# kshedden/muscato

Hardware: AMD Instinct MI355X
Metric: reads/sec (100 bp, multi-map) at 1/2/4/8 MI355X; confirm-kernel HBM GB/s vs peak (higher is better)
Workload: dtype u32

## Files before the change

muscato_amd/build.py:

```python
from __future__ import annotations

import os
import shutil
import subprocess
from concurrent.futures import ThreadPoolExecutor

HERE = os.path.dirname(os.path.abspath(__file__))
CSRC = os.path.join(HERE, "csrc")
LIB = os.path.join(HERE, "libmuscato_hip.so")
OBJ = os.path.join(HERE, "build")
SOURCES = [os.path.join(CSRC, f) for f in ("muscato_hip.hip", "match_lane_rw4.hip", "match_lane_rw8.hip", "match_lane_rw12.hip",
                                           "match_lane_rw8w.hip", "match_lane_rw12w.hip", "match_lane_rw16w.hip", "match_lane_rw8s.hip", "match_dma_rw8.hip")]
HEADERS = [os.path.join(os.path.dirname(HERE), "include", "muscato_hip.h")] + \
    [os.path.join(CSRC, f) for f in sorted(os.listdir(CSRC)) if f.endswith(".hpp")]
LANE_ONLY = os.path.join(CSRC, "kernels_match_lane.hpp")
DMA_ONLY = os.path.join(CSRC, "kernels_match_dma.hpp")
FLAGS = ["--offload-arch=gfx950", "-O3", "-std=c++17", "-fPIC", "-Wall", "-Wno-unused-function"]


def hipcc() -> str:
    for cand in (shutil.which("hipcc"), "/opt/rocm/bin/hipcc"):
        if cand and os.path.exists(cand):
            return cand
    raise RuntimeError("hipcc not found: libmuscato_hip.so cannot be built")


def needs_build() -> bool:
    if not os.path.exists(LIB):
        return True
    t = os.path.getmtime(LIB)
    return any(os.path.getmtime(p) > t for p in SOURCES + HEADERS)


HOST = os.path.join(CSRC, "host")
BIN = os.path.join(HERE, "bin")
HOST_HEADERS = [os.path.join(HOST, f) for f in sorted(os.listdir(HOST)) if f.endswith(".hpp")]
TOOLS = {"muscato": "muscato_cli.cpp", "muscato_prep_targets": "muscato_prep_targets.cpp",
         "muscato_screen": "muscato_screen.cpp", "muscato_confirm": "muscato_confirm.cpp"}
GPU_TOOLS = ("muscato", "muscato_prep_targets", "muscato_screen", "muscato_confirm")


def build_tools(force: bool = False, verbose: bool = False) -> None:
    os.makedirs(BIN, exist_ok=True)
    for name, src in TOOLS.items():
        out = os.path.join(BIN, name)
        srcp = os.path.join(HOST, src)
        deps = [srcp] + HOST_HEADERS + HEADERS
        if not force and os.path.exists(out) and all(os.path.getmtime(d) <= os.path.getmtime(out) for d in deps):
            continue
        cmd = ["g++", "-O2", "-std=c++17", "-Wall", "-pthread", "-o", out, srcp, "-lz"]
        if name in GPU_TOOLS:
            cmd += ["-L" + HERE, "-lmuscato_hip", "-Wl,-rpath,$ORIGIN/.."]
        if verbose:
            print(" ".join(cmd))
        subprocess.check_call(cmd)


_API = "../../include/muscato_hip.h"
_HOST_CHAIN = ("host/muscato_host.hpp", "host/cli_config.hpp", "host/cli_maxmatches_host.hpp", "host/cli_names.hpp", "host/cli_plan.hpp",
               "host/cli_text.hpp", "host/sz.hpp", _API)
CHECKS = {
    "cli_plan_check": ("cli_plan_check.cpp", ("host/check.hpp", "host/cli_names.hpp", "host/cli_plan.hpp"), 83_615_609, ()),
    "ctx_state_check": ("ctx_state_check.cpp", ("host/check.hpp", "ctx_state.hpp", _API), 58_376_821, ()),
    "dev_mem_check": ("dev_mem_check.cpp", ("host/check.hpp", "dev_mem.hpp"), 492, ()),
    "index_plan_check": ("index_plan_check.cpp", ("host/check.hpp", "index_plan.hpp"), 567_030, ()),
    "load_plan_check": ("load_plan_check.cpp", ("host/check.hpp", "load_plan.hpp"), 35_240_767, ()),
    "maxmatches_plan_check": ("maxmatches_plan_check.cpp", ("host/check.hpp", "maxmatches_plan.hpp"), 548_365, ()),
    "read_names_plan_check": ("read_names_plan_check.cpp", ("host/check.hpp", "read_names_plan.hpp"), 21_577_989, ()),
    "side_names_check": ("side_names_check.cpp", ("host/check.hpp", "side_names.hpp"), 100_517, ()),
    "sz_plan_check": ("sz_plan_check.cpp", ("host/check.hpp", "sz_plan.hpp", "host/sz.hpp"), 3_599_466, ("-lz",)),
    "targets_prep_plan_check": ("targets_prep_plan_check.cpp", ("host/check.hpp", "sz_plan.hpp", "targets_prep_plan.hpp") + _HOST_CHAIN, 12_757_977, ("-lz",)),
    "text_stage_check": ("text_stage_check.cpp", ("host/check.hpp", "text_stage.hpp"), 1_711_086, ()),
}
SANITIZE = ["-O1", "-g", "-fsanitize=address,undefined", "-fno-sanitize-recover=all", "-static-libasan", "-static-libubsan"]


def check_headers(name: str) -> list:
    return [os.path.normpath(os.path.join(CSRC, h)) for h in CHECKS[name][1]]


def build_checks(force: bool = False, verbose: bool = False, sanitize: bool = False, out_dir: str = BIN) -> dict:
    os.makedirs(out_dir, exist_ok=True)

    def one(name: str) -> str:
        src, _, _, libs = CHECKS[name]
        out = os.path.join(out_dir, name + ("_san" if sanitize else ""))
        srcp = os.path.join(HOST, src)
        deps = [srcp] + check_headers(name)
        if force or not os.path.exists(out) or any(os.path.getmtime(d) > os.path.getmtime(out) for d in deps):
            cmd = ["g++", "-std=c++17", "-Wall"] + (SANITIZE if sanitize else ["-O2"]) + ["-o", out, srcp] + list(libs)
            if verbose:
                print(" ".join(cmd))
            subprocess.check_call(cmd)
        return out

    with ThreadPoolExecutor(max_workers=len(CHECKS)) as ex:
        return dict(zip(CHECKS, ex.map(one, CHECKS)))


def _compile(src: str, force: bool, verbose: bool, defines=(), tag: str = "") -> str:
    obj = os.path.join(OBJ, os.path.basename(src) + tag + ".o")
    base = os.path.basename(src)
    deps = [src] + [h for h in HEADERS if (h != LANE_ONLY or "match_lane" in base or "match_dma" in base) and (h != DMA_ONLY or "match_dma" in base)]
    if not force and os.path.exists(obj) and all(os.path.getmtime(d) <= os.path.getmtime(obj) for d in deps):
        return obj
    cmd = [hipcc()] + FLAGS + list(defines) + ["-c", "-o", obj, src]
    if verbose:
        print(" ".join(cmd))
    subprocess.check_call(cmd)
    return obj


def build(force: bool = False, verbose: bool = False) -> str:
    if force or needs_build():
        os.makedirs(OBJ, exist_ok=True)
        with ThreadPoolExecutor(max_workers=len(SOURCES)) as ex:
            objs = list(ex.map(lambda s: _compile(s, force, verbose), SOURCES))
        cmd = [hipcc(), "--offload-arch=gfx950", "-shared", "-fPIC", "-o", LIB] + objs + ["-ldl"]
        if verbose:
            print(" ".join(cmd))
        subprocess.check_call(cmd)
    build_tools(force=force, verbose=verbose)
    build_checks(force=force, verbose=verbose)
    return LIB


def variant(name: str, defines) -> str:
    os.makedirs(OBJ, exist_ok=True)
    out_dir = os.path.join(os.path.dirname(HERE), "build_variants")
    os.makedirs(out_dir, exist_ok=True)
    with ThreadPoolExecutor(max_workers=len(SOURCES)) as ex:
        main_defs = ["-D" + d[len("-DMAIN_"):] for d in defines if d.startswith("-DMAIN_")]
        lane_defs = [d for d in defines if not d.startswith("-DMAIN_")]
        objs = list(ex.map(lambda s: _compile(s, False, False, lane_defs if ("match_lane" in s or "match_dma" in s) else main_defs,
                                              "." + name if (("match_lane" in s or "match_dma" in s) and lane_defs) or ("match_lane" not in s and "match_dma" not in s and main_defs) else ""), SOURCES))
    out = os.path.join(out_dir, name + ".so")
    subprocess.check_call([hipcc(), "--offload-arch=gfx950", "-shared", "-fPIC", "-o", out] + objs + ["-ldl"])
    return out


if __name__ == "__main__":
    import sys
    if len(sys.argv) > 2 and sys.argv[1] == "variant":
        print(variant(sys.argv[2], sys.argv[3:]))
    else:
        print(build(force="--force" in sys.argv, verbose=True))
```

muscato_amd/csrc/muscato_hip.hip:

```cpp

#include <hip/hip_runtime.h>
#include <rccl/rccl.h>
#include <dlfcn.h>

#include <algorithm>
#include <cstdarg>
#include <cstdio>
#include <cstdlib>
#include <cstring>
#include <map>
#include <mutex>
#include <string>
#include <type_traits>
#include <vector>

#include "../../include/muscato_hip.h"

#include "ctx_state.hpp"
#include "dev_mem.hpp"
#include "index_plan.hpp"
#include "load_plan.hpp"

#include "kernels_common.hpp"
#include "kernels_index.hpp"
#include "kernels_screen.hpp"
#include "kernels_confirm.hpp"
#include "kernels_match.hpp"
#include "kernels_match_lane_inst.hpp"
#include "kernels_screen_lane.hpp"
#include "kernels_partition.hpp"
#include "kernels_results.hpp"
#include "side_names.hpp"
#include "kernels_side.hpp"
#include "kernels_maxmatches.hpp"
#include "kernels_fastq.hpp"
MUSC_LANE_INSTANCES_4(extern)
MUSC_LANE_INSTANCES_8(extern)
MUSC_LANE_INSTANCES_12(extern)
MUSC_LANE_INSTANCES_8W(extern)
MUSC_LANE_INSTANCES_12W(extern)
MUSC_LANE_INSTANCES_16W(extern)
MUSC_LANE_INSTANCES_SPEC(extern)
MUSC_DMA_INSTANCES(extern)


namespace {

thread_local std::string g_init_error;

struct Roctx {
  int (*push)(const char*) = nullptr;
  int (*pop)() = nullptr;
  Roctx() {
    for (const char* name : {"librocprofiler-sdk-roctx.so.1", "librocprofiler-sdk-roctx.so", "libroctx64.so.4", "libroctx64.so"}) {
      if (void* h = dlopen(name, RTLD_NOW | RTLD_LOCAL)) {
        push = reinterpret_cast<int (*)(const char*)>(dlsym(h, "roctxRangePushA"));
        pop = reinterpret_cast<int (*)()>(dlsym(h, "roctxRangePop"));
        if (push && pop) return;
        push = nullptr;
        pop = nullptr;
      }
    }
  }
};
const Roctx& roctx() {
  static const Roctx r;
  return r;
}
struct Range {
  bool on;
  explicit Range(const char* name) : on(roctx().push != nullptr) {
    if (on) (void)roctx().push(name);
  }
  ~Range() {
    if (on) (void)roctx().pop();
  }
};

struct CaptureGuard {
  hipStream_t st = nullptr;
  bool active = false;
  hipError_t begin(hipStream_t s) {
    const hipError_t e = hipStreamBeginCapture(s, hipStreamCaptureModeThreadLocal);
    if (e == hipSuccess) {
      st = s;
      active = true;
    }
    return e;
  }
  hipError_t end(hipGraph_t* g) {
    active = false;
    return hipStreamEndCapture(st, g);
  }
  ~CaptureGuard() {
    if (!active) return;
    hipGraph_t g = nullptr;
    (void)hipStreamEndCapture(st, &g);
    if (g) (void)hipGraphDestroy(g);
    (void)hipGetLastError();
  }
};

}

using musc_load::RecShape;
using musc_load::StreamPlan;
using musc_load::stream_plan;
using musc_load::stream_plan_batch;

struct EnvKnobs : musc_index::Knobs {
  bool match_dma = false;
  bool screen_wg = false;
  int context = 0;
  bool no_x_context = false;
  bool force_wide = false;
  int debug_grid = 0;
  bool debug_sync = false;
  int graph = -1;
  bool pipeline = false;
  bool no_spec = false;
  long batch_reads = 0;
  uint64_t stage_bytes = 64ull << 20;
  uint64_t stage_lines = 1ull << 20;
  long mm_heap_lds = 0;
  void read() {
    *this = EnvKnobs();
    auto is = [](const char* v, const char* w) { return v && !strcmp(v, w); };
    const char* e = getenv("MUSC_INDEX");
    index = is(e, "classic") ? musc_index::IDX_CLASSIC : is(e, "lines") ? musc_index::IDX_LINES : is(e, "classic64") ? musc_index::IDX_CLASSIC64 : musc_index::IDX_AUTO;
    e = getenv("MUSC_MATCH");
    match_dma = is(e, "dma");
    screen_wg = is(getenv("MUSC_SCREEN"), "wg");
    e = getenv("MUSC_CONTEXT");
    context = is(e, "narrow") ? 1 : is(e, "wide") ? 2 : 0;
    no_x_context = getenv("MUSC_NO_X_CONTEXT") != nullptr;
    force_wide = getenv("MUSC_DEBUG_FORCE_WIDE") != nullptr;
    if ((e = getenv("MUSC_DEBUG_INDEX_BITS"))) index_bits = atoi(e);
    ctx_direct = (e = getenv("MUSC_DEBUG_CTX_DIRECT")) && atoi(e) > 0;
    if ((e = getenv("MUSC_DEBUG_GRID"))) debug_grid = atoi(e);
    debug_sync = getenv("MUSC_DEBUG_SYNC") != nullptr;
    if ((e = getenv("MUSC_GRAPH"))) graph = atoi(e);
    if ((e = getenv("MUSC_PIPELINE"))) pipeline = atoi(e) > 0;
    no_spec = getenv("MUSC_NO_SPEC") != nullptr;
    if ((e = getenv("MUSC_BATCH_READS"))) batch_reads = atol(e);
    if ((e = getenv("MUSC_DEBUG_INDEX_BUDGET_MB"))) index_budget_mb = atol(e);
    if ((e = getenv("MUSC_DEBUG_STAGE_BYTES")) && atoll(e) > 0) stage_bytes = (uint64_t)atoll(e);
    if ((e = getenv("MUSC_DEBUG_STAGE_LINES")) && atoll(e) > 0) stage_lines = (uint64_t)atoll(e);
    if ((e = getenv("MUSC_DEBUG_MM_HEAP_LDS"))) mm_heap_lds = atol(e);
  }
};

struct musc_ctx {
  int device = 0;
  hipStream_t stream = nullptr;
  std::string err;
  EnvKnobs env;
  musc_state::State st;

  DevPtr<uint32_t> db2;
  DevPtr<uint32_t> dbm2;
  bool db_has_x = false;
  bool reads_have_x = false;
  DevBuf<uint32_t> rdx;
  struct { uint64_t gen = 0; int wide = -1; } rdx_of;
  struct { uint64_t gen = 0; double pmatch = -1.0; int32_t mmp1 = -1; bool ok = false; } xok;
  DevPtr<uint32_t> dbx;
  uint64_t max_tlen = 0;
  struct { uint64_t gen = 0; int32_t key[CTX_MAX_W + 3] = {0}; bool ok = false; } xokdb;
  DevPtr<uint64_t> seq_off;
  uint32_t nseq = 0;
  uint64_t nbases = 0;
  uint64_t db_words = 0;
  std::vector<uint64_t> h_seq_off;

  uint64_t part_bases = 0;
  std::vector<uint32_t> part_first;
  musc_index::Kind part_kind = musc_index::K_CLASSIC64;
  uint64_t part_size = 0;
  uint32_t cur_part = 0;
  DevBuf<musc_hit> pacc;
  DevBuf<uint32_t> pbest;
  DevBuf<uint64_t> pcnt, padj;
  DevBuf<uint32_t> pflags, pflags_tmp;
  DevBuf<uint32_t> block_acc;

  musc_index::Resident idx;
  int wide = 0;
  DevMem idx_T, idx_E, ctx_T, ctx_E;
  unsigned scrt_resident = 0;
  int scrt_rw = 0;
  uint64_t idx_novf = 0;
  DevPtr<PathParams> d_pp;
  PathParams h_pp;
  bool h_pp_valid = false;
  DevPtr<MatchParams> d_mp;
  MatchParams h_mp;
  bool h_mp_valid = false;
  int spec_geom = 0;
  DevBuf<uint4> spill;

  DevPtr<uint32_t> rd;
  uint64_t rd_cap = 0;
  DevPtr<uint32_t> rdm;
  uint64_t nreads = 0;
  int rw = 0;
  uint32_t max_len = 0;
  bool reads_failed = false;

  struct Upload {
    DevPtr<uint32_t> stage;
    hipStream_t s_up = nullptr;
    std::vector<hipEvent_t> ev;
    StreamPlan plan;
    uint64_t next_piece = 0;
    uint64_t packed_upto = 0;
    uint32_t L = 0;
    bool active = false;
  } up;

  struct BatchSet {
    DevBuf<uint32_t> wb, rvalid, tbase, tcount;
    DevBuf<uint4> cdesc;
  } bs[2];
  int cur = 0;
  hipStream_t stream2 = nullptr;
  hipStream_t s_confirm = nullptr;
  hipEvent_t ev_ready[2] = {nullptr, nullptr}, ev_free[2] = {nullptr, nullptr}, ev_join = nullptr;
  DevBuf<uint32_t> scan_tmp, tcount2, tpre;
  DevBuf<uint4> stage;
  DevBuf<uint32_t> p_nx;
  DevBuf<uint16_t> nmiss_tab;
// ... 1004 lines not shown
```

muscato_amd/csrc/muscato_prep.hpp:

```cpp

#include <rocprim/device/device_radix_sort.hpp>

#define PREP_BASES_PER_WORD 21

DEV uint32_t prep_code(unsigned char ch) {
  switch (ch) {
    case 'A': return 1u;
    case 'C': return 2u;
    case 'G': return 3u;
    case 'T': return 4u;
    default: return 5u;
  }
}

MUSC_KERNEL __launch_bounds__(256) void k_prep_keys(const unsigned char* __restrict__ s,
                                                   const uint64_t* __restrict__ off,
                                                   const uint32_t* __restrict__ perm, uint64_t n, uint32_t w,
                                                   uint64_t* __restrict__ keys) {
  for (uint64_t i = (uint64_t)blockIdx.x * blockDim.x + threadIdx.x; i < n; i += (uint64_t)gridDim.x * blockDim.x) {
    const uint32_t r = perm[i];
    const uint64_t o = off[r];
    const uint64_t len = off[r + 1] - o;
    const uint64_t first = (uint64_t)w * PREP_BASES_PER_WORD;
    uint64_t key = 0;
    for (uint32_t j = 0; j < PREP_BASES_PER_WORD; j++) {
      const uint64_t q = first + j;
      if (q >= len) break;
      key |= (uint64_t)prep_code(s[o + q]) << (60 - 3 * j);
    }
    keys[i] = key;
  }
}

MUSC_KERNEL void k_prep_iota(uint32_t* __restrict__ p, uint64_t n) {
  for (uint64_t i = (uint64_t)blockIdx.x * blockDim.x + threadIdx.x; i < n; i += (uint64_t)gridDim.x * blockDim.x)
    p[i] = (uint32_t)i;
}

MUSC_KERNEL __launch_bounds__(256) void k_prep_heads(const unsigned char* __restrict__ s,
                                                    const uint64_t* __restrict__ off,
                                                    const uint32_t* __restrict__ perm, uint64_t n,
                                                    uint32_t* __restrict__ head) {
  for (uint64_t i = (uint64_t)blockIdx.x * blockDim.x + threadIdx.x; i < n; i += (uint64_t)gridDim.x * blockDim.x) {
    uint32_t h = 1;
    if (i > 0) {
      const uint32_t a = perm[i], b = perm[i - 1];
      const uint64_t oa = off[a], ob = off[b];
      const uint64_t la = off[a + 1] - oa, lb = off[b + 1] - ob;
      if (la == lb) {
        h = 0;
        for (uint64_t q = 0; q < la; q++)
          if (s[oa + q] != s[ob + q]) {
            h = 1;
            break;
          }
      }
    }
    head[i] = h;
  }
}

MUSC_KERNEL void k_prep_starts(const uint32_t* __restrict__ head, const uint32_t* __restrict__ incl, uint64_t n,
                              uint32_t* __restrict__ ustart, uint32_t* __restrict__ uhead,
                              const uint32_t* __restrict__ perm) {
  for (uint64_t i = (uint64_t)blockIdx.x * blockDim.x + threadIdx.x; i < n; i += (uint64_t)gridDim.x * blockDim.x) {
    if (head[i]) {
      ustart[incl[i] - 1] = (uint32_t)i;
      uhead[incl[i] - 1] = perm[i];
    }
    if (i == n - 1) ustart[incl[i]] = (uint32_t)n;
  }
}

MUSC_KERNEL void k_prep_pack(const unsigned char* __restrict__ s, const uint64_t* __restrict__ off,
                            const uint32_t* __restrict__ uhead, uint64_t nunique, int rw,
                            uint32_t* __restrict__ rd, uint32_t* __restrict__ rdm, uint32_t* __restrict__ has_x) {
  const uint64_t t = (uint64_t)blockIdx.x * blockDim.x + threadIdx.x;
  const uint64_t g = t / rw;
  const int j = (int)(t % rw);
  if (g >= nunique) return;
  const uint32_t r = uhead[g];
  const uint64_t o = off[r];
  const uint32_t len = (uint32_t)(off[r + 1] - o);
  if (j == rw - 1) {
    uint32_t anyx = 0;
    for (uint32_t q = 0; q < len; q++) {
      uint32_t isx;
      (void)ascii_code(s[o + q], &isx);
      anyx |= isx;
    }
    rd[t] = (len & 0xFFFFu) | (anyx ? READ_HAS_X : 0u);
    rdm[t] = 0;
    return;
  }
  uint32_t v = 0, mv = 0;
  for (int b = 0; b < 16; b++) {
    const uint32_t q = (uint32_t)j * 16 + b;
    if (q < len) {
      uint32_t isx;
      const uint32_t c = ascii_code(s[o + q], &isx);
      v |= c << (2 * b);
      mv |= isx << (2 * b);
    }
  }
  rd[t] = v;
  rdm[t] = mv;
  if (mv) atomicOr(has_x, 1u);
}

static int reads_sort_unique_dev(musc_ctx* c, const char* who, const unsigned char* d_s, const uint64_t* d_off, const uint64_t n,
                                 const Marks& m, uint32_t** order, uint32_t** ustart, uint64_t* nunique) {
  TmpBufs B;
  RecShape shape;
  uint64_t first = 0, last = 0, maxlen = 0;
  int rc = offsets_census(c, d_off, n, &first, &last, &maxlen);
  if (rc) return rc;
  if (first != 0) return fail(c, 2, "read offsets[0] must be 0");
  if ((rc = reads_shape(c, 0, maxlen, false, &shape))) return rc;

  const uint32_t nw = (uint32_t)std::max<uint64_t>((maxlen + PREP_BASES_PER_WORD - 1) / PREP_BASES_PER_WORD, 1);
  uint64_t *k0 = nullptr, *k1 = nullptr;
  uint32_t *p0 = nullptr, *p1 = nullptr;
  if ((rc = tmp_alloc(c, who, B, &k0, n * 8)) || (rc = tmp_alloc(c, who, B, &k1, n * 8)) || (rc = tmp_alloc(c, who, B, &p0, n * 4)) ||
      (rc = tmp_alloc(c, who, B, &p1, n * 4)))
    return rc;
  size_t tmp_bytes = 0;
  HIPCHK(c, rocprim::radix_sort_pairs(nullptr, tmp_bytes, k0, k1, p0, p1, (size_t)n, 0u, 63u, c->stream));
  void* tmp = nullptr;
  if ((rc = tmp_alloc(c, who, B, &tmp, tmp_bytes))) return rc;
  const dim3 grid(std::min(nblk(n, 256), MAX_GRID));
  hipLaunchKernelGGL(k_prep_iota, grid, dim3(256), 0, c->stream, p0, n);
  HIPCHK(c, hipGetLastError());
  for (uint32_t w = nw; w-- > 0;) {
    hipLaunchKernelGGL(k_prep_keys, grid, dim3(256), 0, c->stream, d_s, d_off, p0, n, w, k0);
    HIPCHK(c, hipGetLastError());
    HIPCHK(c, rocprim::radix_sort_pairs(tmp, tmp_bytes, k0, k1, p0, p1, (size_t)n, 0u, 63u, c->stream));
    std::swap(p0, p1);
  }

  uint32_t *head = nullptr, *incl = nullptr, *stmp = nullptr, *d_ustart = nullptr, *d_uhead = nullptr;
  if ((rc = tmp_alloc(c, who, B, &head, n * 4)) || (rc = tmp_alloc(c, who, B, &incl, n * 4)) ||
      (rc = tmp_alloc(c, who, B, &stmp, scan_tmp_elems(n) * 4)) || (rc = tmp_alloc(c, who, B, &d_ustart, (n + 1) * 4)) ||
      (rc = tmp_alloc(c, who, B, &d_uhead, n * 4)))
    return rc;
  hipLaunchKernelGGL(k_prep_heads, grid, dim3(256), 0, c->stream, d_s, d_off, p0, n, head);
  HIPCHK(c, hipGetLastError());
  if ((rc = scan_u32(c, head, incl, n, true, stmp))) return rc;
  hipLaunchKernelGGL(k_prep_starts, grid, dim3(256), 0, c->stream, head, incl, n, d_ustart, d_uhead, p0);
  HIPCHK(c, hipGetLastError());
  uint32_t nu32 = 0;
  HIPCHK(c, hipMemcpyAsync(&nu32, incl + (n - 1), 4, hipMemcpyDeviceToHost, c->stream));
  HIPCHK(c, hipStreamSynchronize(c->stream));
  const uint64_t nu = nu32;

  if ((rc = reads_shape(c, nu, maxlen, false, &shape)) || (rc = reads_records(c, shape, nu, maxlen, true, false))) return rc;
  const auto [rw, words] = shape;
  uint32_t* d_hasx = c->d_flag;
  HIPCHK(c, hipMemsetAsync(d_hasx, 0, 4, c->stream));
  hipLaunchKernelGGL(k_prep_pack, dim3(nblk(words, 256)), dim3(256), 0, c->stream, d_s, d_off, d_uhead, nu, rw, c->rd,
                     c->rdm, d_hasx);
  HIPCHK(c, hipGetLastError());
  HIPCHK(c, m.mark(c, 1));

  uint32_t* h_order = (uint32_t*)malloc(n * 4);
  uint32_t* h_ustart = (uint32_t*)malloc((nu + 1) * 4);
  if (!h_order || !h_ustart) {
    free(h_order);
    free(h_ustart);
    return fail(c, 7, "out of host memory for the sort order");
  }
  uint32_t hasx = 0;
  hipError_t e = hipMemcpyAsync(h_order, p0, n * 4, hipMemcpyDeviceToHost, c->stream);
  if (e == hipSuccess) e = hipMemcpyAsync(h_ustart, d_ustart, (nu + 1) * 4, hipMemcpyDeviceToHost, c->stream);
  if (e == hipSuccess) e = hipMemcpyAsync(&hasx, d_hasx, 4, hipMemcpyDeviceToHost, c->stream);
  if (e == hipSuccess) e = hipStreamSynchronize(c->stream);
  if (e != hipSuccess) {
    free(h_order);
    free(h_ustart);
    return fail(c, 10, "musc_reads_sort_unique: %s", hipGetErrorString(e));
  }
  reads_settle_x(c, hasx);
  c->stats.ms_read_prep = m.ms(0, 1);
  *order = h_order;
  *ustart = h_ustart;
  *nunique = nu;
  return 0;
}

static int reads_sort_unique_run(musc_ctx* c, const char* seqs, const uint64_t* offsets, uint64_t nreads, int on_device,
                                 uint32_t** order, uint32_t** ustart, uint64_t* nunique) {
  HIPCHK(c, hipSetDevice(c->device));
  free_reads(c);
  if (nreads >= 0xFFFFFFF0ull) return fail(c, 2, "too many reads for 32-bit read numbers");
  if (nreads == 0) {
    c->rw = 4;
    *order = (uint32_t*)malloc(4);
    *ustart = (uint32_t*)calloc(1, 4);
    if (!*order || !*ustart) return fail(c, 7, "out of host memory");
    return 0;
  }
  static const char* const who = "musc_reads_sort_unique";
  Marks m;
  int rc = m.start(c);
  if (rc) return rc;
  TmpBufs B;
  const unsigned char* d_s = nullptr;
  const uint64_t* d_off = nullptr;
  if ((rc = staged(c, who, B, (const unsigned char*)seqs, on_device ? 0 : offsets[nreads], on_device, 64, &d_s)) ||
      (rc = staged(c, who, B, offsets, (nreads + 1) * 8, on_device, 0, &d_off)))
    return rc;
  HIPCHK(c, m.mark(c, 0));
  return reads_sort_unique_dev(c, who, d_s, d_off, nreads, m, order, ustart, nunique);
}

extern "C" int musc_reads_sort_unique(musc_ctx* c, const char* seqs, const uint64_t* offsets, uint64_t nreads,
                                      int on_device, uint32_t** order, uint32_t** ustart, uint64_t* nunique) {
  if (!c) return 1;
  if (!order || !ustart || !nunique) return fail(c, 2, "musc_reads_sort_unique: NULL output pointer");
  *order = *ustart = nullptr;
  *nunique = 0;
  if ((!seqs || !offsets) && nreads) return fail(c, 2, "musc_reads_sort_unique: NULL input");
  return reads_load_done(c, reads_sort_unique_run(c, seqs, offsets, nreads, on_device, order, ustart, nunique));
}


extern "C" void musc_fastq_prep_free(musc_fastq_prep* p) {
  if (!p) return;
  free(p->name_off);
  free(p->seq_off);
  free(p->name_len);
  free(p->seq_len);
  free(p->order);
  free(p->ustart);
  memset(p, 0, sizeof *p);
}

static int fastq_prep_run(musc_ctx* c, const char* text, uint64_t nbytes, int on_device, int32_t min_len, uint32_t max_len,
                          musc_fastq_prep* out) {
  static const char* const who = "musc_reads_prep_fastq";
  Marks m;
  int rc = m.start(c);
  if (rc) return rc;
  TmpBufs P;
  TmpBufs S;
  const unsigned char* d_text = nullptr;
  if ((rc = staged(c, who, P, (const unsigned char*)text, nbytes, on_device, 16, &d_text))) return rc;
  HIPCHK(c, m.mark(c, 0));

  TextLines L;
  if (nbytes && (rc = text_lines(c, who, P, d_text, nbytes, &L))) return rc;
  const uint64_t nrec = (L.newlines + L.virt) / 4;
  if (nrec >= 0xFFFFFFF0ull) return fail(c, 2, "too many reads for 32-bit read numbers");

  uint64_t *lines = nullptr, *len = nullptr;
  uint32_t *kidx = nullptr, *name_len = nullptr;
  uint64_t nkept = 0, total = 0;
  if (nrec) {
// ... 74 lines not shown
```

Baseline: 2.100 billion.

## Encode reads once into key planes and records before sorting unique reads

Result: no change. 2.104 billion, median of 4 (+0.2%).

```diff
diff --git a/muscato_amd/build.py b/muscato_amd/build.py
--- a/muscato_amd/build.py
+++ b/muscato_amd/build.py
@@ -72,18 +72,22 @@
     "targets_prep_plan_check": ("targets_prep_plan_check.cpp", ("host/check.hpp", "sz_plan.hpp", "targets_prep_plan.hpp") + _HOST_CHAIN, 12_757_977, ("-lz",)),
     "text_stage_check": ("text_stage_check.cpp", ("host/check.hpp", "text_stage.hpp"), 1_711_086, ()),
 }
+MORE_CHECKS = {
+    "prep_encode_verify": ("prep_encode_verify.cpp", ("host/check.hpp", "prep_encode.hpp"), 5_784_897, ()),
+}
 SANITIZE = ["-O1", "-g", "-fsanitize=address,undefined", "-fno-sanitize-recover=all", "-static-libasan", "-static-libubsan"]
 
 
 def check_headers(name: str) -> list:
-    return [os.path.normpath(os.path.join(CSRC, h)) for h in CHECKS[name][1]]
+    return [os.path.normpath(os.path.join(CSRC, h)) for h in {**CHECKS, **MORE_CHECKS}[name][1]]
 
 
-def build_checks(force: bool = False, verbose: bool = False, sanitize: bool = False, out_dir: str = BIN) -> dict:
+def build_checks(force: bool = False, verbose: bool = False, sanitize: bool = False, out_dir: str = BIN, table: dict = None) -> dict:
+    table = CHECKS if table is None else table
     os.makedirs(out_dir, exist_ok=True)
 
     def one(name: str) -> str:
-        src, _, _, libs = CHECKS[name]
+        src, _, _, libs = table[name]
         out = os.path.join(out_dir, name + ("_san" if sanitize else ""))
         srcp = os.path.join(HOST, src)
         deps = [srcp] + check_headers(name)
@@ -94,8 +98,8 @@
             subprocess.check_call(cmd)
         return out
 
-    with ThreadPoolExecutor(max_workers=len(CHECKS)) as ex:
-        return dict(zip(CHECKS, ex.map(one, CHECKS)))
+    with ThreadPoolExecutor(max_workers=len(table)) as ex:
+        return dict(zip(table, ex.map(one, table)))
 
 
 def _compile(src: str, force: bool, verbose: bool, defines=(), tag: str = "") -> str:
@@ -122,6 +126,7 @@
         subprocess.check_call(cmd)
     build_tools(force=force, verbose=verbose)
     build_checks(force=force, verbose=verbose)
+    build_checks(force=force, verbose=verbose, table=MORE_CHECKS)
     return LIB
 
 
diff --git a/muscato_amd/csrc/host/prep_encode_verify.cpp b/muscato_amd/csrc/host/prep_encode_verify.cpp
--- /dev/null
+++ b/muscato_amd/csrc/host/prep_encode_verify.cpp
@@ -0,0 +1,197 @@
+#include <algorithm>
+#include <cstdint>
+#include <cstring>
+#include <string>
+#include <vector>
+
+#include "../prep_encode.hpp"
+#include "check.hpp"
+
+using namespace musc_prep;
+
+namespace {
+
+struct Text {
+  std::vector<uint32_t> words;
+  uint64_t t0 = 0, t1 = 0;
+  static constexpr uint64_t BASE = 0x7000;
+  Text(const std::string& s, uint32_t lead) {
+    const size_t bytes = (lead + s.size() + 3 + 16) & ~(size_t)3;
+    words.assign(bytes / 4, 0x54545454u);
+    memcpy(reinterpret_cast<unsigned char*>(words.data()) + lead, s.data(), s.size());
+    t0 = BASE + lead;
+    t1 = t0 + s.size();
+  }
+  uint32_t load(uint64_t a) const {
+    EXPECT_MSG((a & 3) == 0 && dword_in_text(a, t0, t1), "load of %llx outside [%llx, %llx)", (unsigned long long)a,
+               (unsigned long long)t0, (unsigned long long)t1);
+    const unsigned char* p = reinterpret_cast<const unsigned char*>(words.data()) + (a - BASE);
+    return (uint32_t)p[0] | ((uint32_t)p[1] << 8) | ((uint32_t)p[2] << 16) | ((uint32_t)p[3] << 24);
+  }
+};
+
+struct Encoded {
+  std::vector<uint64_t> key;
+  std::vector<uint32_t> rec, mask;
+  uint32_t flags = 0;
+  uint64_t loads = 0;
+};
+
+Encoded walk(const Text& T, uint64_t o, uint32_t len, uint32_t nw, uint32_t rw) {
+  Encoded E;
+  E.key.assign(nw, ~0ull);
+  E.rec.assign(rw, ~0u);
+  E.mask.assign(rw, ~0u);
+  std::vector<uint32_t> L(TILE_DWORDS, 0xA5A5A5A5u), Enc(TILE_ENC, 0x5A5A5A5Au);
+  const uint32_t ntiles = (len + TILE_BASES - 1) / TILE_BASES;
+  uint32_t anyx = 0;
+  for (uint32_t t = 0; t < ntiles; t++) {
+    const uint32_t q0 = t * TILE_BASES, nbt = std::min(len - q0, TILE_BASES);
+    const uint64_t addr = T.t0 + o + q0, a0 = span_first(addr);
+    const uint32_t sh = span_shift(addr), need = span_count(addr, nbt);
+    EXPECT(need <= TILE_DWORDS - 2);
+    for (uint32_t i = 0; i < need; i++) {
+      const uint64_t a = a0 + 4ull * i;
+      if (dword_in_text(a, T.t0, T.t1)) {
+        L[i] = T.load(a);
+        E.loads++;
+      } else {
+        L[i] = 0;
+      }
+    }
+    for (uint32_t d = 0; 4 * d < nbt; d++) {
+      uint32_t odd;
+      EXPECT(d + 1 < TILE_DWORDS && d < TILE_ENC);
+      Enc[d] = encode4(align_bytes(L[d], L[d + 1], sh), &odd);
+      if (odd_of(odd, nbt - 4 * d)) E.flags |= FLAG_NON_ACGTX;
+    }
+    for (uint32_t k = 0; k < TILE_KEYS; k++) {
+      const uint32_t w = t * TILE_KEYS + k;
+      if (w >= nw) break;
+      const uint32_t nb = word_bases(nbt, k, KEY_BASES);
+      EXPECT(((KEY_BASES * k) >> 2) + KEY_WINDOW <= TILE_ENC);
+      E.key[w] = nb ? key_word(Enc.data(), KEY_BASES * k, nb) : 0;
+    }
+    for (uint32_t k = 0; k < TILE_RECS; k++) {
+      const uint32_t j = t * TILE_RECS + k;
+      if (j + 1 >= rw) break;
+      const uint32_t nb = word_bases(nbt, k, REC_BASES);
+      uint32_t v = 0, mv = 0;
+      if (nb) rec_word(Enc.data(), k, nb, &v, &mv);
+      E.rec[j] = v;
+      E.mask[j] = mv;
+      anyx |= mv;
+    }
+  }
+  if (anyx) E.flags |= FLAG_NON_ACGT;
+  for (uint32_t w = ntiles * TILE_KEYS; w < nw; w++) E.key[w] = 0;
+  for (uint32_t j = ntiles * TILE_RECS; j + 1 < rw; j++) E.rec[j] = E.mask[j] = 0;
+  E.rec[rw - 1] = (len & 0xFFFFu) | (anyx ? 0x10000u : 0u);
+  E.mask[rw - 1] = 0;
+  return E;
+}
+
+Encoded bytewise(const std::string& s, uint32_t nw, uint32_t rw) {
+  Encoded E;
+  E.key.assign(nw, 0);
+  E.rec.assign(rw, 0);
+  E.mask.assign(rw, 0);
+  uint32_t anyx = 0;
+  for (size_t q = 0; q < s.size(); q++) {
+    const unsigned char ch = (unsigned char)s[q];
+    const bool acgt = ch == 'A' || ch == 'C' || ch == 'G' || ch == 'T';
+    const uint64_t k3 = ch == 'A' ? 1 : ch == 'C' ? 2 : ch == 'G' ? 3 : ch == 'T' ? 4 : 5;
+    const uint32_t c2 = ch == 'C' ? 1 : ch == 'G' ? 2 : ch == 'T' ? 3 : 0;
+    E.key[q / 21] |= k3 << (60 - 3 * (q % 21));
+    E.rec[q / 16] |= c2 << (2 * (q % 16));
+    if (!acgt) {
+      E.mask[q / 16] |= 1u << (2 * (q % 16));
+      anyx = 1;
+      E.flags |= FLAG_NON_ACGT;
+      if (ch != 'X') E.flags |= FLAG_NON_ACGTX;
+    }
+  }
+  E.rec[rw - 1] = ((uint32_t)s.size() & 0xFFFFu) | (anyx ? 0x10000u : 0u);
+  return E;
+}
+
+uint32_t rw_for(uint32_t maxlen) { return ((maxlen + 15) / 16 + 1 + 3) & ~3u; }
+
+uint64_t g_state = 0x9E3779B97F4A7C15ull;
+uint32_t rnd() {
+  g_state ^= g_state << 13;
+  g_state ^= g_state >> 7;
+  g_state ^= g_state << 17;
+  return (uint32_t)(g_state >> 32);
+}
+
+std::string random_read(uint32_t len, const char* alphabet, uint32_t na) {
+  std::string s(len, 'A');
+  for (auto& ch : s) ch = alphabet[rnd() % na];
+  return s;
+}
+
+void one_case(const std::string& read, uint32_t before, uint32_t after, uint32_t lead, uint32_t maxlen) {
+  const uint32_t nw = std::max<uint32_t>((maxlen + 20) / 21, 1), rw = rw_for(maxlen);
+  const std::string text = std::string(before, 'G') + read + std::string(after, 'C');
+  const Text T(text, lead);
+  const Encoded got = walk(T, before, (uint32_t)read.size(), nw, rw), want = bytewise(read, nw, rw);
+  EXPECT_MSG(got.key == want.key, "keys: len %zu before %u after %u lead %u maxlen %u", read.size(), before, after, lead, maxlen);
+  EXPECT_MSG(got.rec == want.rec, "record: len %zu before %u after %u lead %u maxlen %u", read.size(), before, after, lead, maxlen);
+  EXPECT_MSG(got.mask == want.mask, "mask: len %zu before %u after %u lead %u maxlen %u", read.size(), before, after, lead, maxlen);
+  EXPECT_MSG(got.flags == want.flags, "flags %u, want %u: len %zu", got.flags, want.flags, read.size());
+  uint64_t most = 0;
+  for (uint32_t q0 = 0; q0 < read.size(); q0 += TILE_BASES)
+    most += span_count(T.t0 + before + q0, std::min<uint32_t>((uint32_t)read.size() - q0, TILE_BASES));
+  EXPECT(got.loads <= most);
+}
+
+}
+
+int main() {
+  EXPECT(span_count(0x1000, 0) == 0 && span_count(0x1003, 1) == 1 && span_count(0x1003, 2) == 2 && span_count(0x1000, 4) == 1);
+  EXPECT(span_count(0x1001, 4) == 2 && span_count(0x1003, TILE_BASES) == 85 && span_first(0x1003) == 0x1000 && span_shift(0x1003) == 3);
+  EXPECT(dword_in_text(0x0FFC, 0x0FFF, 0x1001) && dword_in_text(0x1000, 0x0FFF, 0x1001) && !dword_in_text(0x1004, 0x0FFF, 0x1001));
+  EXPECT(!dword_in_text(0x0FF8, 0x0FFF, 0x1001) && !dword_in_text(0x1000, 0x1000, 0x1000));
+  EXPECT(word_bases(100, 4, 21) == 16 && word_bases(100, 5, 21) == 0 && word_bases(105, 4, 21) == 21 && word_bases(0, 0, 16) == 0);
+  EXPECT(align_bytes(0x44332211u, 0x88776655u, 0) == 0x44332211u && align_bytes(0x44332211u, 0x88776655u, 1) == 0x55443322u &&
+         align_bytes(0x44332211u, 0x88776655u, 3) == 0x77665544u);
+
+  for (uint32_t place = 0; place < 4; place++)
+    for (uint32_t ch = 0; ch < 256; ch++)
+      for (uint32_t others : {0x41414141u, 0x54475443u, 0x58585858u, 0x00FF6E4Eu, 0xFFFFFFFFu, 0u}) {
+        const uint32_t v = (others & ~(0xFFu << (8 * place))) | (ch << (8 * place));
+        uint32_t odd, want_c2 = 0, want_m = 0, want_k = 0, want_odd = 0;
+        const uint32_t e = encode4(v, &odd);
+        for (uint32_t b = 0; b < 4; b++) {
+          const uint32_t c = (v >> (8 * b)) & 0xFFu;
+          const uint32_t c2 = c == 'C' ? 1 : c == 'G' ? 2 : c == 'T' ? 3 : 0, acgt = c == 'A' || c2;
+          want_c2 |= c2 << (2 * b);
+          want_m |= (acgt ? 0u : 1u) << (2 * b);
+          want_k |= (acgt ? c2 + 1 : 5u) << (9 - 3 * b);
+          want_odd |= (acgt || c == 'X' ? 0u : 0x80u) << (8 * b);
+        }
+        EXPECT_MSG(e == (want_c2 | (want_m << 8) | (want_k << 16)) && odd == want_odd, "encode4(%08x) = %08x, odd %08x", v, e, odd);
+      }
+
+  static const char ACGT[] = "ACGT", ACGTX[] = "ACGTX", ANY[] = {'A', 'C', 'G', 'T', 'X', 'N', 'a', 't', '\0', (char)0xFF, 'B', 'U'};
+  std::vector<uint32_t> lens;
+  for (uint32_t l = 0; l <= 130; l++) lens.push_back(l);
+  for (uint32_t l : {314u, 315u, 316u, 319u, 320u, 321u, 335u, 336u, 337u, 338u, 352u, 357u, 671u, 672u, 673u, 1000u, 1008u, 1009u})
+    lens.push_back(l);
+  for (uint32_t len : lens)
+    for (uint32_t lead = 0; lead < 16; lead++)
+      for (uint32_t before : {0u, 1u, 2u, 3u, 5u})
+        for (uint32_t after : {0u, 1u, 7u}) {
+          const std::string r = random_read(len, (len + lead) % 3 == 0 ? ACGT : (len + lead) % 3 == 1 ? ACGTX : ANY,
+                                            (len + lead) % 3 == 0 ? 4 : (len + lead) % 3 == 1 ? 5 : 12);
+          one_case(r, before, after, lead, len);
+          one_case(r, before, after, lead, len + 1 + rnd() % 700);
+        }
+  for (uint32_t lead : {0u, 1u, 2u, 3u}) {
+    one_case(random_read(65535, ACGTX, 5), 3, 0, lead, 65535);
+    one_case(random_read(65534, ACGT, 4), 0, 2, lead, 65535);
+    one_case(random_read(17, ANY, 12), 1, 0, lead, 65535);
+  }
+  return check_done("prep_encode_verify");
+}
diff --git a/muscato_amd/csrc/kernels_prep.hpp b/muscato_amd/csrc/kernels_prep.hpp
--- /dev/null
+++ b/muscato_amd/csrc/kernels_prep.hpp
@@ -0,0 +1,129 @@
+#pragma once
+#include "prep_encode.hpp"
+
+#define PE_GROUP 8u
+
+DEV void pe_group_sync() {
+  __builtin_amdgcn_fence(__ATOMIC_RELEASE, "wavefront");
+  __builtin_amdgcn_wave_barrier();
+  __builtin_amdgcn_fence(__ATOMIC_ACQUIRE, "wavefront");
+}
+
+MUSC_KERNEL __launch_bounds__(256) void k_prep_encode(const unsigned char* __restrict__ s, const uint64_t* __restrict__ off,
+                                                     uint64_t n, uint64_t total, uint32_t nw, uint32_t rw,
+                                                     uint64_t* __restrict__ K, uint32_t* __restrict__ R,
+                                                     uint32_t* __restrict__ M, uint32_t* __restrict__ flags) {
+  using namespace musc_prep;
+  __shared__ uint32_t s_img[256 / PE_GROUP][TILE_DWORDS];
+  __shared__ uint32_t s_enc[256 / PE_GROUP][TILE_ENC];
+  const uint32_t sub = threadIdx.x & (PE_GROUP - 1u);
+  uint32_t* const L = s_img[threadIdx.x / PE_GROUP];
+  uint32_t* const E = s_enc[threadIdx.x / PE_GROUP];
+  const uint64_t t0 = (uint64_t)(uintptr_t)s, t1 = t0 + total;
+  const uint64_t ngroups = (uint64_t)gridDim.x * (256 / PE_GROUP);
+  uint32_t fl = 0;
+  uint64_t r = (uint64_t)blockIdx.x * (256 / PE_GROUP) + threadIdx.x / PE_GROUP;
+  uint64_t o_next = r < n ? off[r] : 0, e_next = r < n ? off[r + 1] : 0;
+  for (; r < n; r += ngroups) {
+    const uint64_t o = o_next;
+    const uint32_t len = (uint32_t)(e_next - o);
+    if (r + ngroups < n) {
+      o_next = off[r + ngroups];
+      e_next = off[r + ngroups + 1];
+    }
+    const uint32_t ntiles = (len + TILE_BASES - 1) / TILE_BASES;
+    uint32_t* const rec = R + r * rw;
+    uint32_t* const mrec = M + r * rw;
+    uint32_t anyx = 0;
+    for (uint32_t t = 0; t < ntiles; t++) {
+      const uint32_t q0 = t * TILE_BASES;
+      const uint32_t nbt = len - q0 < TILE_BASES ? len - q0 : TILE_BASES;
+      const uint64_t addr = t0 + o + q0, a0 = span_first(addr);
+      const uint32_t sh = span_shift(addr), need = span_count(addr, nbt);
+      pe_group_sync();
+      for (uint32_t i = sub; i < need; i += PE_GROUP) {
+        const uint64_t a = a0 + 4ull * i;
+        L[i] = dword_in_text(a, t0, t1) ? *reinterpret_cast<const uint32_t*>((uintptr_t)a) : 0u;
+      }
+      pe_group_sync();
+      for (uint32_t d = sub; 4 * d < nbt; d += PE_GROUP) {
+        uint32_t odd;
+        E[d] = encode4(align_bytes(L[d], L[d + 1], sh), &odd);
+        if (odd_of(odd, nbt - 4 * d)) fl |= FLAG_NON_ACGTX;
+      }
+      pe_group_sync();
+      for (uint32_t k = sub; k < TILE_KEYS; k += PE_GROUP) {
+        const uint32_t w = t * TILE_KEYS + k;
+        if (w >= nw) break;
+        const uint32_t nb = word_bases(nbt, k, KEY_BASES);
+        K[(uint64_t)w * n + r] = nb ? key_word(E, KEY_BASES * k, nb) : 0;
+      }
+      for (uint32_t k = sub; k < TILE_RECS; k += PE_GROUP) {
+        const uint32_t j = t * TILE_RECS + k;
+        if (j + 1 >= rw) break;
+        const uint32_t nb = word_bases(nbt, k, REC_BASES);
+        uint32_t v = 0, mv = 0;
+        if (nb) rec_word(E, k, nb, &v, &mv);
+        rec[j] = v;
+        mrec[j] = mv;
+        anyx |= mv;
+      }
+    }
+    for (uint32_t w = ntiles * TILE_KEYS + sub; w < nw; w += PE_GROUP) K[(uint64_t)w * n + r] = 0;
+    for (uint32_t j = ntiles * TILE_RECS + sub; j + 1 < rw; j += PE_GROUP) {
+      rec[j] = 0;
+      mrec[j] = 0;
+    }
+#pragma unroll
+    for (uint32_t d = 1; d < PE_GROUP; d <<= 1) anyx |= __shfl_xor(anyx, d);
+    if (sub == 0) {
+      rec[rw - 1] = (len & 0xFFFFu) | (anyx ? READ_HAS_X : 0u);
+      mrec[rw - 1] = 0;
+    }
+    if (anyx) fl |= FLAG_NON_ACGT;
+  }
+  if (fl) atomicOr(flags, fl);
+}
+
+MUSC_KERNEL __launch_bounds__(256) void k_prep_gather(const uint64_t* __restrict__ plane, const uint32_t* __restrict__ perm,
+                                                     uint64_t n, uint64_t* __restrict__ keys) {
+  for (uint64_t i = (uint64_t)blockIdx.x * blockDim.x + threadIdx.x; i < n; i += (uint64_t)gridDim.x * blockDim.x)
+    keys[i] = plane[perm[i]];
+}
+
+MUSC_KERNEL __launch_bounds__(256) void k_prep_heads_keys(const uint64_t* __restrict__ k0s, const uint64_t* __restrict__ K,
+                                                         const uint32_t* __restrict__ perm, uint64_t n, uint32_t nw,
+                                                         const unsigned char* __restrict__ s, const uint64_t* __restrict__ off,
+                                                         const uint32_t* __restrict__ flags, uint32_t* __restrict__ head) {
+  const bool bytes = (*flags & musc_prep::FLAG_NON_ACGTX) != 0;
+  for (uint64_t i = (uint64_t)blockIdx.x * blockDim.x + threadIdx.x; i < n; i += (uint64_t)gridDim.x * blockDim.x) {
+    uint32_t h = 1;
+    if (i > 0 && k0s[i] == k0s[i - 1]) {
+      const uint32_t a = perm[i], b = perm[i - 1];
+      h = 0;
+      for (uint32_t w = 1; w < nw; w++)
+        if (K[(uint64_t)w * n + a] != K[(uint64_t)w * n + b]) {
+          h = 1;
+          break;
+        }
+      if (!h && bytes) {
+        const uint64_t oa = off[a], ob = off[b];
+        const uint64_t la = off[a + 1] - oa;
+        for (uint64_t q = 0; q < la; q++)
+          if (s[oa + q] != s[ob + q]) {
+            h = 1;
+            break;
+          }
+      }
+    }
+    head[i] = h;
+  }
+}
+
+MUSC_KERNEL __launch_bounds__(256) void k_prep_copy(const uint4* __restrict__ src, const uint32_t* __restrict__ uhead,
+                                                   uint64_t nunique, uint32_t q, uint4* __restrict__ dst) {
+  const uint64_t t = (uint64_t)blockIdx.x * blockDim.x + threadIdx.x;
+  const uint64_t g = t / q;
+  if (g >= nunique) return;
+  dst[t] = src[(uint64_t)uhead[g] * q + (t - g * q)];
+}
diff --git a/muscato_amd/csrc/muscato_hip.hip b/muscato_amd/csrc/muscato_hip.hip
--- a/muscato_amd/csrc/muscato_hip.hip
+++ b/muscato_amd/csrc/muscato_hip.hip
@@ -34,6 +34,7 @@
 #include "kernels_side.hpp"
 #include "kernels_maxmatches.hpp"
 #include "kernels_fastq.hpp"
+#include "kernels_prep.hpp"
 MUSC_LANE_INSTANCES_4(extern)
 MUSC_LANE_INSTANCES_8(extern)
 MUSC_LANE_INSTANCES_12(extern)
@@ -123,6 +124,8 @@
   uint64_t stage_bytes = 64ull << 20;
   uint64_t stage_lines = 1ull << 20;
   long mm_heap_lds = 0;
+  bool prep_encode = true;
+  long prep_plane_mb = -1;
   void read() {
     *this = EnvKnobs();
     auto is = [](const char* v, const char* w) { return v && !strcmp(v, w); };
@@ -147,6 +150,8 @@
     if ((e = getenv("MUSC_DEBUG_STAGE_BYTES")) && atoll(e) > 0) stage_bytes = (uint64_t)atoll(e);
     if ((e = getenv("MUSC_DEBUG_STAGE_LINES")) && atoll(e) > 0) stage_lines = (uint64_t)atoll(e);
     if ((e = getenv("MUSC_DEBUG_MM_HEAP_LDS"))) mm_heap_lds = atol(e);
+    prep_encode = !is(getenv("MUSC_PREP_ENCODE"), "0");
+    if ((e = getenv("MUSC_DEBUG_PREP_PLANE_MB")) && atol(e) >= 0) prep_plane_mb = atol(e);
   }
 };
 
diff --git a/muscato_amd/csrc/muscato_prep.hpp b/muscato_amd/csrc/muscato_prep.hpp
--- a/muscato_amd/csrc/muscato_prep.hpp
+++ b/muscato_amd/csrc/muscato_prep.hpp
@@ -32,7 +32,8 @@
   }
 }
 
-MUSC_KERNEL void k_prep_iota(uint32_t* __restrict__ p, uint64_t n) {
+MUSC_KERNEL void k_prep_iota(uint32_t* __restrict__ p, uint64_t n, uint32_t* __restrict__ zero) {
+  if (zero && blockIdx.x == 0 && threadIdx.x == 0) *zero = 0;
   for (uint64_t i = (uint64_t)blockIdx.x * blockDim.x + threadIdx.x; i < n; i += (uint64_t)gridDim.x * blockDim.x)
     p[i] = (uint32_t)i;
 }
@@ -108,9 +109,33 @@
   if (mv) atomicOr(has_x, 1u);
 }
 
+struct PrepPlanes {
+  uint64_t* K = nullptr;
+  uint32_t *R = nullptr, *M = nullptr;
+};
+static bool prep_planes_alloc(musc_ctx* c, TmpBufs& EK, TmpBufs& E, uint64_t n, uint32_t nw, int rw, PrepPlanes* P) {
+  if (!c->env.prep_encode) return false;
+  const uint64_t kbytes = (uint64_t)nw * n * 8, rbytes = n * (uint64_t)rw * 4;
+  const uint64_t planes = kbytes + 2 * rbytes;
+  if (c->env.prep_plane_mb >= 0 && planes > ((uint64_t)c->env.prep_plane_mb << 20)) return false;
+  size_t free_b = 0, total_b = 0;
+  if (hipMemGetInfo(&free_b, &total_b) != hipSuccess) {
+    (void)hipGetLastError();
+    return false;
+  }
+  if ((uint64_t)free_b < planes + 2 * (rbytes + 256) + (64ull << 20)) return false;
+  if (EK.alloc(&P->K, kbytes) != hipSuccess || E.alloc(&P->R, rbytes) != hipSuccess || E.alloc(&P->M, rbytes) != hipSuccess) {
+    (void)hipGetLastError();
+    EK.release();
+    E.release();
+    return false;
+  }
+  return true;
+}
+
 static int reads_sort_unique_dev(musc_ctx* c, const char* who, const unsigned char* d_s, const uint64_t* d_off, const uint64_t n,
                                  const Marks& m, uint32_t** order, uint32_t** ustart, uint64_t* nunique) {
-  TmpBufs B;
+  TmpBufs B, EK, E;
   RecShape shape;
   uint64_t first = 0, last = 0, maxlen = 0;
   int rc = offsets_census(c, d_off, n, &first, &last, &maxlen);
@@ -121,44 +146,66 @@
   const uint32_t nw = (uint32_t)std::max<uint64_t>((maxlen + PREP_BASES_PER_WORD - 1) / PREP_BASES_PER_WORD, 1);
   uint64_t *k0 = nullptr, *k1 = nullptr;
   uint32_t *p0 = nullptr, *p1 = nullptr;
+  uint32_t *head = nullptr, *incl = nullptr, *stmp = nullptr, *d_ustart = nullptr, *d_uhead = nullptr;
   if ((rc = tmp_alloc(c, who, B, &k0, n * 8)) || (rc = tmp_alloc(c, who, B, &k1, n * 8)) || (rc = tmp_alloc(c, who, B, &p0, n * 4)) ||
       (rc = tmp_alloc(c, who, B, &p1, n * 4)))
     return rc;
   size_t tmp_bytes = 0;
   HIPCHK(c, rocprim::radix_sort_pairs(nullptr, tmp_bytes, k0, k1, p0, p1, (size_t)n, 0u, 63u, c->stream));
   void* tmp = nullptr;
-  if ((rc = tmp_alloc(c, who, B, &tmp, tmp_bytes))) return rc;
-  const dim3 grid(std::min(nblk(n, 256), MAX_GRID));
-  hipLaunchKernelGGL(k_prep_iota, grid, dim3(256), 0, c->stream, p0, n);
-  HIPCHK(c, hipGetLastError());
-  for (uint32_t w = nw; w-- > 0;) {
-    hipLaunchKernelGGL(k_prep_keys, grid, dim3(256), 0, c->stream, d_s, d_off, p0, n, w, k0);
-    HIPCHK(c, hipGetLastError());
-    HIPCHK(c, rocprim::radix_sort_pairs(tmp, tmp_bytes, k0, k1, p0, p1, (size_t)n, 0u, 63u, c->stream));
-    std::swap(p0, p1);
-  }
-
-  uint32_t *head = nullptr, *incl = nullptr, *stmp = nullptr, *d_ustart = nullptr, *d_uhead = nullptr;
-  if ((rc = tmp_alloc(c, who, B, &head, n * 4)) || (rc = tmp_alloc(c, who, B, &incl, n * 4)) ||
+  if ((rc = tmp_alloc(c, who, B, &tmp, tmp_bytes)) || (rc = tmp_alloc(c, who, B, &head, n * 4)) || (rc = tmp_alloc(c, who, B, &incl, n * 4)) ||
       (rc = tmp_alloc(c, who, B, &stmp, scan_tmp_elems(n) * 4)) || (rc = tmp_alloc(c, who, B, &d_ustart, (n + 1) * 4)) ||
       (rc = tmp_alloc(c, who, B, &d_uhead, n * 4)))
     return rc;
-  hipLaunchKernelGGL(k_prep_heads, grid, dim3(256), 0, c->stream, d_s, d_off, p0, n, head);
+  PrepPlanes P;
+  const bool enc = prep_planes_alloc(c, EK, E, n, nw, shape.rw, &P);
+  uint32_t* const d_flags = c->d_flag;
+
+  const dim3 grid(std::min(nblk(n, 256), MAX_GRID));
+  hipLaunchKernelGGL(k_prep_iota, grid, dim3(256), 0, c->stream, p0, n, enc ? d_flags : (uint32_t*)nullptr);
+  HIPCHK(c, hipGetLastError());
+  if (enc) {
+    hipLaunchKernelGGL(k_prep_encode, dim3(std::min(nblk(n, 256 / PE_GROUP), 4 * MAX_GRID)), dim3(256), 0, c->stream, d_s, d_off, n, last,
+                       nw, (uint32_t)shape.rw, P.K, P.R, P.M, d_flags);
+    HIPCHK(c, hipGetLastError());
+  }
+  for (uint32_t w = nw; w-- > 0;) {
+    uint64_t* kin = k0;
+    if (!enc) hipLaunchKernelGGL(k_prep_keys, grid, dim3(256), 0, c->stream, d_s, d_off, p0, n, w, k0);
+    else if (w == nw - 1) kin = P.K + (uint64_t)w * n;
+    else hipLaunchKernelGGL(k_prep_gather, grid, dim3(256), 0, c->stream, P.K + (uint64_t)w * n, p0, n, k0);
+    HIPCHK(c, hipGetLastError());
+    HIPCHK(c, rocprim::radix_sort_pairs(tmp, tmp_bytes, kin, k1, p0, p1, (size_t)n, 0u, 63u, c->stream));
+    std::swap(p0, p1);
+  }
+
+  if (enc) hipLaunchKernelGGL(k_prep_heads_keys, grid, dim3(256), 0, c->stream, k1, P.K, p0, n, nw, d_s, d_off, d_flags, head);
+  else hipLaunchKernelGGL(k_prep_heads, grid, dim3(256), 0, c->stream, d_s, d_off, p0, n, head);
   HIPCHK(c, hipGetLastError());
   if ((rc = scan_u32(c, head, incl, n, true, stmp))) return rc;
   hipLaunchKernelGGL(k_prep_starts, grid, dim3(256), 0, c->stream, head, incl, n, d_ustart, d_uhead, p0);
   HIPCHK(c, hipGetLastError());
-  uint32_t nu32 = 0;
+  uint32_t nu32 = 0, flags = 0;
   HIPCHK(c, hipMemcpyAsync(&nu32, incl + (n - 1), 4, hipMemcpyDeviceToHost, c->stream));
+  if (enc) HIPCHK(c, hipMemcpyAsync(&flags, d_flags, 4, hipMemcpyDeviceToHost, c->stream));
   HIPCHK(c, hipStreamSynchronize(c->stream));
   const uint64_t nu = nu32;
-
-  if ((rc = reads_shape(c, nu, maxlen, false, &shape)) || (rc = reads_records(c, shape, nu, maxlen, true, false))) return rc;
+  EK.release();
+
+  const bool mask = !enc || (flags & musc_prep::FLAG_NON_ACGT);
+  if ((rc = reads_shape(c, nu, maxlen, false, &shape)) || (rc = reads_records(c, shape, nu, maxlen, mask, false))) return rc;
   const auto [rw, words] = shape;
-  uint32_t* d_hasx = c->d_flag;
-  HIPCHK(c, hipMemsetAsync(d_hasx, 0, 4, c->stream));
-  hipLaunchKernelGGL(k_prep_pack, dim3(nblk(words, 256)), dim3(256), 0, c->stream, d_s, d_off, d_uhead, nu, rw, c->rd,
-                     c->rdm, d_hasx);
+  if (enc) {
+    const uint32_t q = (uint32_t)rw / 4;
+    hipLaunchKernelGGL(k_prep_copy, dim3(nblk(nu * q, 256)), dim3(256), 0, c->stream, reinterpret_cast<const uint4*>(P.R), d_uhead, nu, q,
+                       reinterpret_cast<uint4*>(c->rd.p));
+    if (mask)
+      hipLaunchKernelGGL(k_prep_copy, dim3(nblk(nu * q, 256)), dim3(256), 0, c->stream, reinterpret_cast<const uint4*>(P.M), d_uhead, nu,
+                         q, reinterpret_cast<uint4*>(c->rdm.p));
+  } else {
+    HIPCHK(c, hipMemsetAsync(d_flags, 0, 4, c->stream));
+    hipLaunchKernelGGL(k_prep_pack, dim3(nblk(words, 256)), dim3(256), 0, c->stream, d_s, d_off, d_uhead, nu, rw, c->rd, c->rdm, d_flags);
+  }
   HIPCHK(c, hipGetLastError());
   HIPCHK(c, m.mark(c, 1));
 
@@ -169,10 +216,10 @@
     free(h_ustart);
     return fail(c, 7, "out of host memory for the sort order");
   }
-  uint32_t hasx = 0;
+  uint32_t hasx = mask;
   hipError_t e = hipMemcpyAsync(h_order, p0, n * 4, hipMemcpyDeviceToHost, c->stream);
   if (e == hipSuccess) e = hipMemcpyAsync(h_ustart, d_ustart, (nu + 1) * 4, hipMemcpyDeviceToHost, c->stream);
-  if (e == hipSuccess) e = hipMemcpyAsync(&hasx, d_hasx, 4, hipMemcpyDeviceToHost, c->stream);
+  if (e == hipSuccess && !enc) e = hipMemcpyAsync(&hasx, d_flags, 4, hipMemcpyDeviceToHost, c->stream);
   if (e == hipSuccess) e = hipStreamSynchronize(c->stream);
   if (e != hipSuccess) {
     free(h_order);
diff --git a/muscato_amd/csrc/prep_encode.hpp b/muscato_amd/csrc/prep_encode.hpp
--- /dev/null
+++ b/muscato_amd/csrc/prep_encode.hpp
@@ -0,0 +1,78 @@
+#pragma once
+#include <cstdint>
+
+#if defined(__HIPCC__)
+#define PE_HD __host__ __device__ inline
+#define PE_UNROLL _Pragma("unroll")
+#else
+#define PE_HD inline
+#define PE_UNROLL
+#endif
+
+namespace musc_prep {
+
+constexpr uint32_t KEY_BASES = 21, REC_BASES = 16;
+constexpr uint32_t TILE_KEYS = 16, TILE_RECS = 21;
+constexpr uint32_t TILE_BASES = KEY_BASES * TILE_KEYS;
+static_assert(TILE_BASES == REC_BASES * TILE_RECS, "a tile holds whole key words and whole record words");
+constexpr uint32_t TILE_DWORDS = 88, TILE_ENC = TILE_BASES / 4;
+constexpr uint32_t KEY_WINDOW = 6;
+
+constexpr uint32_t FLAG_NON_ACGT = 1;
+constexpr uint32_t FLAG_NON_ACGTX = 2;
+
+PE_HD uint64_t span_first(uint64_t addr) { return addr & ~3ull; }
+PE_HD uint32_t span_shift(uint64_t addr) { return (uint32_t)(addr & 3u); }
+PE_HD uint32_t span_count(uint64_t addr, uint32_t nbytes) { return nbytes ? (span_shift(addr) + nbytes + 3u) >> 2 : 0u; }
+PE_HD bool dword_in_text(uint64_t a, uint64_t t0, uint64_t t1) { return a + 4 > t0 && a < t1; }
+
+PE_HD uint32_t align_bytes(uint32_t lo, uint32_t hi, uint32_t sh) {
+#if defined(__HIP_DEVICE_COMPILE__)
+  return __builtin_amdgcn_alignbyte(hi, lo, sh);
+#else
+  return sh ? (lo >> (8 * sh)) | (hi << (32 - 8 * sh)) : lo;
+#endif
+}
+
+PE_HD uint32_t eq_bytes(uint32_t v, uint32_t c4) {
+  const uint32_t x = v ^ c4;
+  return ~(((x & 0x7F7F7F7Fu) + 0x7F7F7F7Fu) | x | 0x7F7F7F7Fu);
+}
+
+PE_HD uint32_t encode4(uint32_t v, uint32_t* odd) {
+  const uint32_t ok = eq_bytes(v, 0x41414141u) | eq_bytes(v, 0x43434343u) | eq_bytes(v, 0x47474747u) | eq_bytes(v, 0x54545454u);
+  *odd = ~(ok | eq_bytes(v, 0x58585858u)) & 0x80808080u;
+  const uint32_t okb = ok >> 7, xb = okb ^ 0x01010101u;
+  uint32_t c = (v >> 1) & 0x03030303u;
+  c = (c ^ ((c >> 1) & 0x01010101u)) & (okb * 3u);
+  const uint32_t c2 = (c | (c >> 6) | (c >> 12) | (c >> 18)) & 0xFFu;
+  const uint32_t m8 = (xb | (xb >> 6) | (xb >> 12) | (xb >> 18)) & 0xFFu;
+  const uint32_t kb = (c + okb) | (xb * 5u);
+  const uint32_t k12 = ((kb << 9) & 0xE00u) | ((kb >> 2) & 0x1C0u) | ((kb >> 13) & 0x038u) | (kb >> 24);
+  return c2 | (m8 << 8) | (k12 << 16);
+}
+PE_HD uint32_t odd_of(uint32_t odd, uint32_t nb) { return nb >= 4 ? odd : odd & ((1u << (8 * nb)) - 1u); }
+
+PE_HD uint64_t key_word(const uint32_t* E, uint32_t f, uint32_t nb) {
+  const uint32_t* e = E + (f >> 2);
+  const uint64_t a = ((uint64_t)((e[0] >> 16) & 0xFFFu) << 48) | ((uint64_t)((e[1] >> 16) & 0xFFFu) << 36) |
+                     ((uint64_t)((e[2] >> 16) & 0xFFFu) << 24) | ((uint64_t)((e[3] >> 16) & 0xFFFu) << 12) |
+                     (uint64_t)((e[4] >> 16) & 0xFFFu);
+  const uint32_t sft = 9 - 3 * (f & 3u);
+  const uint64_t key = ((a << (12 - sft)) | (uint64_t)(((e[5] >> 16) & 0xFFFu) >> sft)) & 0x7FFFFFFFFFFFFFFFull;
+  return key & (~0ull << (63 - 3 * nb));
+}
+
+PE_HD void rec_word(const uint32_t* E, uint32_t k, uint32_t nb, uint32_t* v, uint32_t* mv) {
+  const uint32_t* e = E + 4 * k;
+  const uint32_t keep = nb >= REC_BASES ? ~0u : (1u << (2 * nb)) - 1u;
+  *v = ((e[0] & 0xFFu) | ((e[1] & 0xFFu) << 8) | ((e[2] & 0xFFu) << 16) | (e[3] << 24)) & keep;
+  *mv = (((e[0] >> 8) & 0xFFu) | (e[1] & 0xFF00u) | ((e[2] & 0xFF00u) << 8) | ((e[3] & 0xFF00u) << 16)) & keep;
+}
+
+PE_HD uint32_t word_bases(uint32_t len, uint32_t k, uint32_t per) {
+  const uint64_t first = (uint64_t)k * per;
+  return first >= len ? 0u : (len - first < per ? (uint32_t)(len - first) : per);
+}
+
+}
diff --git a/profiles/read_prep.py b/profiles/read_prep.py
--- /dev/null
+++ b/profiles/read_prep.py
@@ -0,0 +1,43 @@
+#!/usr/bin/env python3
+import json
+import os
+import sys
+
+ROOT = os.path.dirname(os.path.dirname(os.path.abspath(__file__)))
+sys.path.insert(0, ROOT)
+
+
+def main():
+    import torch
+    from muscato_amd import Engine, synth
+
+    wl = synth.workload_for(sys.argv[1] if len(sys.argv) > 1 else "cfg3", 1)
+    if len(sys.argv) > 2 and int(sys.argv[2]):
+        wl = synth.Workload(**{**wl.__dict__, "n_raw_reads": int(sys.argv[2]), "total_raw_reads": None})
+    warm = int(sys.argv[3]) if len(sys.argv) > 3 else 3
+    device = torch.device("cuda", 0)
+    torch.cuda.set_device(0)
+    seed = synth.SEED_BASE + sum(ord(c) for c in wl.seed_key)
+    targets = synth.gen_targets(wl, device, seed)
+    U, n_raw = wl.n_unique_reads, wl.n_raw_reads
+    reads = synth.sort_reads(synth.gen_unique_reads(wl, targets, device, seed + 7919))
+    del targets
+    g = torch.Generator(device=device)
+    g.manual_seed(seed + 17)
+    extra = torch.randint(0, U, (n_raw - U,), device=device, generator=g)
+    raw = torch.cat([reads, reads[extra]])[torch.randperm(n_raw, device=device, generator=g)]
+    del extra, reads
+    raw_off = synth.offsets_for(n_raw, wl.read_len, device)
+    torch.cuda.synchronize()
+    with Engine(0) as eng:
+        for i in range(1 + warm):
+            order, ustart = eng.sort_unique_reads_arrays(raw.data_ptr(), raw_off.data_ptr(), n_raw, True)
+            print(json.dumps({"call": i, "cold": i == 0, "raw_reads": n_raw, "distinct": int(len(ustart) - 1),
+                              "ms_read_prep": eng.stats()["ms_read_prep"],
+                              "encode_path": os.environ.get("MUSC_PREP_ENCODE", "1") != "0"}), flush=True)
+            del order, ustart
+    return 0
+
+
+if __name__ == "__main__":
+    sys.exit(main())
```
